# smups/rustronomy-watershed

Hardware: AMD Instinct MI355X
Metric: Mpixels/s segmenting watershed, 8192x8192 u8, device-resident (throughput, 4 transforms of distinct fields in flight; one transform alone: value_one_transform_alone) (higher is better)
Workload: dtype u8 image / u32 stamps+labels (integer min/max/compare); 1 GPU; 8192x8192 u8 uniform[0,254) random field per GPU, segmenting transform, max_water_level 254, seeds = find_local_minima (7320260 on rank 0's first field), engine fused; 4 contexts in flight, each transforming ITS OWN field and seed list (generator seeds 1..4); parallelism=independent fields x1, world_size=1, devices_visible=1, fields_per_gpu=1

## Files before the change

rustronomy-watershed_amd/csrc/ws_common.hpp:

```cpp
#pragma once

#include <hip/hip_runtime.h>
#include <stdint.h>
#include <stdlib.h>

namespace wsk {

#ifdef WS_TUNING
inline const char *tuning_env(const char *name) { return getenv(name); }
#else
inline const char *tuning_env(const char *) { return nullptr; }
#endif

constexpr uint32_t KEY_INF = 0xFF000000u;
constexpr uint32_t RING_MASK = 0x00FFFFFFu;

constexpr int TS = 64;
constexpr int LP = TS + 2;
constexpr int STRIP = 16;
constexpr int NTHREADS = 256;

constexpr int COUNTER_RING = 64;
constexpr int NSTRIPE = 64;
constexpr int STRIPE_STRIDE = 16;
constexpr int FLAG_SLOT = NSTRIPE * STRIPE_STRIDE;

#ifdef __HIPCC__
__device__ __forceinline__ uint32_t wave_inclusive_sum(uint32_t v) {
#define WS_DPP_ADD(ctrl, rows) v += (uint32_t)__builtin_amdgcn_update_dpp(0, (int)v, ctrl, rows, 0xF, false)
  WS_DPP_ADD(0x111, 0xF);
  WS_DPP_ADD(0x112, 0xF);
  WS_DPP_ADD(0x114, 0xF);
  WS_DPP_ADD(0x118, 0xF);
  WS_DPP_ADD(0x142, 0xA);
  WS_DPP_ADD(0x143, 0xC);
#undef WS_DPP_ADD
  return v;
}

__device__ __forceinline__ uint32_t xcd_span_index(uint32_t b, uint32_t n) {
  constexpr uint32_t XCDS = 8;
  const uint32_t per = n / XCDS;
  return b < per * XCDS ? (b % XCDS) * per + b / XCDS : b;
}

__device__ __forceinline__ size_t padded_img_index(int gy, int gx, int W, int SH, size_t stride) {
  const int slice = gy / SH, ry = gy - slice * SH;
  const int iy = max(min(max(ry, 1), SH - 2) - 1, 0), ix = max(min(max(gx, 1), W - 2) - 1, 0);
  return ((size_t)slice * (size_t)max(SH - 2, 0) + iy) * stride + ix;
}
#endif

struct PassFlags {
  uint32_t *edge_changed;
  uint32_t *any_change;
  uint32_t *overflow;
  uint32_t *stats;
};

hipError_t fill_u32(hipStream_t s, uint32_t *p, size_t n, uint32_t v);
hipError_t words_to_host(hipStream_t s, const uint32_t *a, uint32_t na, uint32_t *host_a, const uint32_t *b, uint32_t nb, uint32_t *host_b);
hipError_t zero3(hipStream_t s, uint32_t *a, size_t na, uint32_t *b, size_t nb, uint32_t *c, size_t nc);
hipError_t random_field(hipStream_t s, uint8_t *img, size_t stride, int h, int w, uint64_t seed);
hipError_t scatter_seeds(hipStream_t s, const uint32_t *seeds_rc, const uint32_t *colours, size_t n, int ph, int pw,
                         uint32_t *labels, uint32_t *keys, uint32_t *err_flag);
hipError_t paint_labels(hipStream_t s, const uint32_t *seeds_rc, size_t n, int ph, int pw, uint32_t *labels,
                        uint32_t *err_flag, uint32_t *zero_a, size_t n_zero_a, uint32_t *zero_b, size_t n_zero_b);
hipError_t seed_tables(hipStream_t s, const uint32_t *seeds_rc, size_t n, int ph, int pw, uint32_t *mask, uint32_t *word_base,
                       uint32_t *err_flag, uint32_t *zero_a, size_t n_zero_a, uint32_t *zero_b, size_t n_zero_b,
                       const uint32_t *slice_first = nullptr, size_t slice_px = 0,
                       uint32_t colour_bias = 0);
hipError_t stack_seeds(hipStream_t s, const uint32_t *seeds_rc, size_t n, const uint32_t *slice_first, size_t n_slices,
                       int slice_h, int pw, uint32_t *stacked_rc, uint32_t shift = 0);
hipError_t narrow_seeds(hipStream_t s, const uint64_t *src, size_t n, size_t ph, size_t pw, uint32_t *dst, uint32_t shift = 0);
hipError_t shift_seeds(hipStream_t s, const uint32_t *src, size_t n, uint32_t shift, uint32_t *dst);
hipError_t widen_labels(hipStream_t s, const uint32_t *src, uint64_t *dst, size_t n);
hipError_t snapshot_level(hipStream_t s, const uint32_t *keys, const uint32_t *labels, uint64_t *dst,
                          size_t n, uint32_t level);
hipError_t snapshot_level_u32(hipStream_t s, const uint32_t *keys, const uint32_t *labels, uint32_t *dst, size_t n, uint32_t level);

size_t relax_tiles(int h, int w);
struct RelaxPlane {
  const uint8_t *img = nullptr;
  size_t img_stride = 0;
  uint32_t *keys = nullptr;
  int h = 0, w = 0;
  uint32_t max_level = 0;
  uint32_t *stamps = nullptr;
  PassFlags pf = {};
  uint32_t max_iters = 0xFFFFFFFFu;
  const uint32_t *seed_labels = nullptr;
  bool seed_bits = false;
  int slice_h = 0;
  bool carry_checked_later = false;
  bool padded = false;
  uint32_t *tile_list = nullptr;
  size_t seam_min_px = (size_t)1 << 24;
  int persistent_pass = 0;
};
hipError_t relax_pass(hipStream_t s, const RelaxPlane &plane, uint32_t pass);
struct RelaxPlan;
RelaxPlan relax_plan_for(const RelaxPlane &plane, uint32_t pass);
size_t relax_list_words(int h, int w);

size_t resolve_tiles(int h, int w);
hipError_t resolve_pass(hipStream_t s, const uint32_t *keys, uint32_t *labels, int h, int w,
                        uint32_t pass, uint32_t *stamps, PassFlags pf);
size_t resolve_ref_capacity(int h, int w);
struct ResolveJob {
  const uint32_t *keys = nullptr;
  uint32_t *labels = nullptr;
  int h = 0, w = 0;
  uint32_t *ref_scratch = nullptr;
  uint32_t max_rounds = 0xFFFFFFFFu;
  const uint32_t *seed_mask = nullptr;
  const uint32_t *word_base = nullptr;
  uint32_t *tile_min = nullptr;
  const uint32_t *gate = nullptr;
  uint32_t *carry_flag = nullptr;
  const uint32_t *seed_err = nullptr;
  int halo_flags = 0;
};
hipError_t resolve_two_launch(hipStream_t s, const ResolveJob &job);
hipError_t resolve_chase_again(hipStream_t s, uint32_t *labels, int h, int w, uint32_t *ref_scratch);

hipError_t block_flag_border_tiles(hipStream_t s, uint32_t *stamps, int h, int w, uint32_t pass, int halo_flags);
hipError_t block_export_boundary(hipStream_t s, const uint32_t *labels, int h, int w, int halo_flags, uint32_t rank, uint32_t *rows);
hipError_t block_import_boundary(hipStream_t s, const uint32_t *table, uint32_t world, uint32_t rank, uint32_t *resolved,
                                 uint32_t *labels, int h, int w, int halo_flags);
hipError_t block_iota(hipStream_t s, uint32_t *p, size_t n, uint32_t first);
hipError_t block_rows_differ(hipStream_t s, const uint32_t *a, const uint32_t *b, size_t n, uint32_t *flag);
hipError_t block_pack_cols(hipStream_t s, const uint32_t *plane, size_t h, size_t w, size_t xl, size_t xr, uint32_t *out);
hipError_t block_unpack_cols(hipStream_t s, uint32_t *plane, size_t h, size_t w, const uint32_t *left, const uint32_t *right);

hipError_t flood_step(hipStream_t s, const uint8_t *img, size_t img_stride, const uint32_t *lin,
                      uint32_t *lout, int h, int w, uint32_t level, uint32_t *counter, bool padded = false);

size_t minima_segments(int h, int w);
size_t minima_mask_bytes(int h, int w);
hipError_t minima_count(hipStream_t s, const uint8_t *img, size_t stride, int h, int w, uint32_t *counts, uint8_t *nibbles);
hipError_t minima_write(hipStream_t s, const uint8_t *nibbles, int h, int w, const uint32_t *counts, uint32_t *total, uint32_t *out_rc, size_t cap,
                        uint32_t *mask = nullptr, uint32_t *word_base = nullptr,
                        uint32_t *zero_a = nullptr, size_t n_zero_a = 0, uint32_t *zero_b = nullptr, size_t n_zero_b = 0);
hipError_t widen_pairs(hipStream_t s, const uint32_t *src, uint64_t *dst, size_t n_values);
hipError_t narrow_words(hipStream_t s, const uint64_t *src, uint32_t *dst, size_t n);

inline int tiles_of(int n) { return (n + TS - 1) / TS; }

}
```

rustronomy-watershed_amd/csrc/ws_kernels.hip:

```cpp
#include "ws_common.hpp"

#include <algorithm>
#include <cstdlib>

namespace wsk {


__global__ void k_fill_u32(uint32_t *p, size_t n, uint32_t v) {
  size_t i = (size_t)blockIdx.x * blockDim.x + threadIdx.x;
  const size_t step = (size_t)gridDim.x * blockDim.x;
  for (; i < n; i += step) p[i] = v;
}

hipError_t fill_u32(hipStream_t s, uint32_t *p, size_t n, uint32_t v) {
  if (n == 0) return hipSuccess;
  const int blocks = (int)((n + 1023) / 1024 < 8192 ? (n + 1023) / 1024 : 8192);
  k_fill_u32<<<blocks, 256, 0, s>>>(p, n, v);
  return hipGetLastError();
}

typedef uint32_t u32x4_z __attribute__((ext_vector_type(4)));
__global__ void k_zero3(uint32_t *a, size_t na, uint32_t *b, size_t nb, uint32_t *c, size_t nc) {
  const size_t tid = (size_t)blockIdx.x * blockDim.x + threadIdx.x, step = (size_t)gridDim.x * blockDim.x;
  size_t head = (size_t)((16u - (unsigned)(reinterpret_cast<uintptr_t>(a) & 15u)) & 15u) >> 2;
// ... 411 lines not shown
}

hipError_t widen_pairs(hipStream_t s, const uint32_t *src, uint64_t *dst, size_t n_values) {
  return widen_labels(s, src, dst, n_values);
}

__global__ void k_narrow_words(const uint64_t *__restrict__ src, uint32_t *__restrict__ dst, size_t n) {
  size_t i = (size_t)blockIdx.x * blockDim.x + threadIdx.x;
  const size_t step = (size_t)gridDim.x * blockDim.x;
  for (; i < n; i += step) dst[i] = (uint32_t)src[i];
}

hipError_t narrow_words(hipStream_t s, const uint64_t *src, uint32_t *dst, size_t n) {
  if (n == 0) return hipSuccess;
  const int blocks = (int)((n + 1023) / 1024 < 8192 ? (n + 1023) / 1024 : 8192);
  k_narrow_words<<<blocks, 256, 0, s>>>(src, dst, n);
  return hipGetLastError();
}

__global__ void k_snapshot(const uint32_t *keys, const uint32_t *labels, uint64_t *dst, size_t n,
                           uint32_t level) {
  size_t i = (size_t)blockIdx.x * blockDim.x + threadIdx.x;
  const size_t step = (size_t)gridDim.x * blockDim.x;
  for (; i < n; i += step) {
    const uint32_t k = keys[i];
    dst[i] = (k != KEY_INF && (k >> 24) <= level) ? (uint64_t)labels[i] : 0ull;
  }
}

__global__ void k_snapshot_u32(const uint32_t *__restrict__ keys, const uint32_t *__restrict__ labels, uint32_t *dst, size_t n, uint32_t level) {
  size_t i = (size_t)blockIdx.x * blockDim.x + threadIdx.x;
  const size_t step = (size_t)gridDim.x * blockDim.x;
  for (; i < n; i += step) {
    const uint32_t k = keys[i];
    dst[i] = (k != KEY_INF && (k >> 24) <= level) ? labels[i] : 0u;
  }
}

hipError_t snapshot_level_u32(hipStream_t s, const uint32_t *keys, const uint32_t *labels, uint32_t *dst, size_t n, uint32_t level) {
  if (n == 0) return hipSuccess;
  const int blocks = (int)((n + 1023) / 1024 < 16384 ? (n + 1023) / 1024 : 16384);
  k_snapshot_u32<<<blocks, 256, 0, s>>>(keys, labels, dst, n, level);
  return hipGetLastError();
}

hipError_t snapshot_level(hipStream_t s, const uint32_t *keys, const uint32_t *labels, uint64_t *dst,
                          size_t n, uint32_t level) {
  if (n == 0) return hipSuccess;
  const int blocks = (int)((n + 1023) / 1024 < 8192 ? (n + 1023) / 1024 : 8192);
  k_snapshot<<<blocks, 256, 0, s>>>(keys, labels, dst, n, level);
  return hipGetLastError();
}

__global__ void k_words_to_host(const uint32_t *__restrict__ a, uint32_t na, uint32_t *ha, const uint32_t *__restrict__ b, uint32_t nb,
                                uint32_t *hb) {
  for (uint32_t i = threadIdx.x; i < na; i += blockDim.x) ha[i] = a[i];
  for (uint32_t i = threadIdx.x; i < nb; i += blockDim.x) hb[i] = b[i];
}

hipError_t words_to_host(hipStream_t s, const uint32_t *a, uint32_t na, uint32_t *host_a, const uint32_t *b, uint32_t nb, uint32_t *host_b) {
  k_words_to_host<<<1, 64, 0, s>>>(a, na, host_a, b, nb, host_b);
  return hipGetLastError();
}

typedef uint32_t u32x4_r __attribute__((ext_vector_type(4)));


__device__ __forceinline__ uint32_t pick_drlu(uint32_t d, uint32_t r, uint32_t l, uint32_t u) {
  return d ? d : (r ? r : (l ? l : u));
}

__global__ __launch_bounds__(256) void k_flood_step(const uint8_t *__restrict__ img, size_t img_stride,
                                                    const uint32_t *__restrict__ lin, uint32_t *__restrict__ lout,
                                                    int H, int W, uint32_t level, uint32_t *counter, int pad) {
  const int x = blockIdx.x * 64 + (threadIdx.x & 63);
  const int y = blockIdx.y * 4 + (threadIdx.x >> 6);
  const int xc = min(x, W - 1), yc = min(y, H - 1);
  const int xm = max(xc - 1, 0), xp = min(xc + 1, W - 1), ym = max(yc - 1, 0), yp = min(yc + 1, H - 1);
  const uint32_t c = lin[(size_t)yc * W + xc];
  const uint32_t d = lin[(size_t)yp * W + xc], r = lin[(size_t)yc * W + xp];
  const uint32_t l = lin[(size_t)yc * W + xm], u = lin[(size_t)ym * W + xc];
  const uint32_t v = img[pad ? padded_img_index(yc, xc, W, H, img_stride) : (size_t)yc * img_stride + xc];
  const bool floodable = c == 0u && y >= 1 && y < H - 1 && x >= 1 && x < W - 1 && v <= level;
  const uint32_t pick = floodable ? pick_drlu(d, r, l, u) : 0u;
  if (x < W && y < H) lout[(size_t)y * W + x] = c ? c : pick;
  if (pick && x < W && y < H) *counter = 1u;
}

__global__ __launch_bounds__(256) void k_flood_step4(const uint8_t *__restrict__ img, size_t img_stride,
                                                     const uint32_t *__restrict__ lin, uint32_t *__restrict__ lout,
                                                     int H, int W, uint32_t level, uint32_t *counter) {
  const int y = blockIdx.y;
  const int x0 = (blockIdx.x * 256 + threadIdx.x) * 4;
  if (x0 >= W) return;
  const int ym = max(y - 1, 0), yp = min(y + 1, H - 1);
  const u32x4_r c = *reinterpret_cast<const u32x4_r *>(lin + (size_t)y * W + x0);
  const u32x4_r dn = *reinterpret_cast<const u32x4_r *>(lin + (size_t)yp * W + x0);
  const u32x4_r up = *reinterpret_cast<const u32x4_r *>(lin + (size_t)ym * W + x0);
  const uint32_t lft = lin[(size_t)y * W + max(x0 - 1, 0)], rgt = lin[(size_t)y * W + min(x0 + 4, W - 1)];
  const uint32_t iv = *reinterpret_cast<const uint32_t *>(img + (size_t)y * img_stride + x0);
  const bool row_int = y >= 1 && y < H - 1;
  const uint32_t cc[4] = {c.x, c.y, c.z, c.w}, dd[4] = {dn.x, dn.y, dn.z, dn.w}, uu[4] = {up.x, up.y, up.z, up.w};
  const uint32_t ll[4] = {lft, c.x, c.y, c.z}, rr[4] = {c.y, c.z, c.w, rgt};
  uint32_t out[4], any = 0;
#pragma unroll
  for (int k = 0; k < 4; ++k) {
    const int x = x0 + k;
    const bool floodable = cc[k] == 0u && row_int && x >= 1 && x < W - 1 && ((iv >> (8 * k)) & 0xFFu) <= level;
    const uint32_t pick = floodable ? pick_drlu(dd[k], rr[k], ll[k], uu[k]) : 0u;
    out[k] = cc[k] ? cc[k] : pick;
    any |= pick;
  }
  *reinterpret_cast<u32x4_r *>(lout + (size_t)y * W + x0) = u32x4_r{out[0], out[1], out[2], out[3]};
  if (any) *counter = 1u;
}

// ... 206 lines not shown
```

rustronomy-watershed_amd/csrc/ws_resolve.hip:

```cpp
#include "ws_common.hpp"
#include "ws_resolve_tile.hpp"

#include <algorithm>

namespace wsk {


__device__ __forceinline__ bool tile_must_run(const uint32_t *stamps_prev, int tx, int ty, int tilesX,
                                              int tilesY, uint32_t pass) {
  if (pass == 0) return true;
  const int t = ty * tilesX + tx;
  bool run = false;
  if (ty > 0) run |= stamps_prev[(size_t)(t - tilesX) * 4 + 1] == pass;
  if (ty + 1 < tilesY) run |= stamps_prev[(size_t)(t + tilesX) * 4 + 0] == pass;
  if (tx > 0) run |= stamps_prev[(size_t)(t - 1) * 4 + 3] == pass;
  if (tx + 1 < tilesX) run |= stamps_prev[(size_t)(t + 1) * 4 + 2] == pass;
  return run;
}

size_t resolve_tiles(int h, int w) { return (size_t)tiles_of(w) * tiles_of(h); }


__global__ __launch_bounds__(NTHREADS) void k_resolve(const uint32_t *__restrict__ keys, uint32_t *labels,
                                                      int H, int W, int tilesX, int tilesY, uint32_t pass,
// ... 82 lines not shown
          if (src) { own[i] = src; sB[ly0 + i][lx] = src; todo &= ~(1u << i); changed = 1; changed_mask |= 1u << i; }
        }
      }
    }
    if (!__syncthreads_or(changed)) break;
  }

  if (gx < W) {
#pragma unroll
    for (int i = 0; i < STRIP; ++i) {
      const int gy = gy0 + i;
      if (((changed_mask >> i) & 1u) && gy < H) labels[(size_t)gy * W + gx] = own[i];
    }
  }
  uint32_t e = 0;
  if (strip == 0 && (changed_mask & 1u)) e |= 1u;
  if (strip == (NTHREADS / 64) - 1 && (changed_mask >> (STRIP - 1))) e |= 2u;
  if (lane == 0 && changed_mask) e |= 4u;
  if (lane == 63 && changed_mask) e |= 8u;
  if (changed_mask) e |= 16u;
  if (e) atomicOr(&s_edges, e);
  __syncthreads();
  if (tid == 0) {
    const uint32_t ed = s_edges;
    if (ed) {
      const size_t t = (size_t)tile_y * tilesX + tile_x;
      if (ed & 1u) stamps_cur[t * 4 + 0] = pass + 1;
      if (ed & 2u) stamps_cur[t * 4 + 1] = pass + 1;
      if (ed & 4u) stamps_cur[t * 4 + 2] = pass + 1;
      if (ed & 8u) stamps_cur[t * 4 + 3] = pass + 1;
      const uint32_t stripe = (blockIdx.x % NSTRIPE) * STRIPE_STRIDE;
      if (ed & 15u) pf.edge_changed[(pass % COUNTER_RING) * FLAG_SLOT + stripe] = 1u;
      pf.any_change[stripe] = 1u;
    }
  }
}

hipError_t resolve_pass(hipStream_t s, const uint32_t *keys, uint32_t *labels, int h, int w,
                        uint32_t pass, uint32_t *stamps, PassFlags pf) {
  const int tx = tiles_of(w), ty = tiles_of(h);
  k_resolve<<<tx * ty, NTHREADS, 0, s>>>(keys, labels, h, w, tx, ty, pass, stamps, pf);
  return hipGetLastError();
}


template <bool TABLES, bool MERGE, bool BLOCK>
__global__ __launch_bounds__(NTHREADS, 5) void k_resolve_local(const uint32_t *__restrict__ keys, uint32_t *labels,
                                                            int H, int W, int tilesX, uint32_t *ref_count,
                                                            uint32_t *ref_list, uint32_t max_rounds,
                                                            const uint32_t *__restrict__ seed_mask,
                                                            const uint32_t *__restrict__ word_base, uint32_t *tile_min,
                                                            const uint32_t *__restrict__ gate, int SH, uint32_t *carry_flag,
                                                            const uint32_t *__restrict__ seed_err, int halo_flags) {
  __shared__ __attribute__((aligned(16))) uint32_t sB[RL_ROWS * RL_P];
  if (TABLES && seed_err && (seed_err[0] | seed_err[2]) != 0u) return;
  if (gate && __builtin_amdgcn_ballot_w64(gate[(threadIdx.x & 63) * STRIPE_STRIDE] != 0u) != 0ull) return;
  const uint32_t tile = xcd_span_index(blockIdx.x, gridDim.x);
  const int tile_x = tile % tilesX, tile_y = tile / tilesX;
  const int tid = threadIdx.x;
  const int lane = tid & 63, wave = tid >> 6;
  const int pc = tid & 15, pr = tid >> 4;
  const int x0 = tile_x * TS, y0 = tile_y * TS;
  const int gx0 = x0 + pc * 4, gy0 = y0 + pr * 4;
  const int lx0 = RL_X0 + pc * 4, ly0 = 1 + pr * 4;
  WS_STAMP(0);

  uint32_t K[4][4], Lb[4][4];
  uint32_t seedbits = 0;
  uint32_t tab_mask[4] = {0u, 0u, 0u, 0u}, tab_base[4] = {0u, 0u, 0u, 0u};
  const bool vec = (W & 3) == 0 && ((reinterpret_cast<uintptr_t>(keys) | reinterpret_cast<uintptr_t>(labels)) & 15u) == 0;
  if (vec) {
    const int gxc = min(gx0, W - 4);
    u32x4_r kv[4], lv[4];
#pragma unroll
    for (int r = 0; r < 4; ++r) {
      const size_t g = (size_t)min(gy0 + r, H - 1) * W + gxc;
      kv[r] = *reinterpret_cast<const u32x4_r *>(keys + g);
      if (TABLES) {
        tab_mask[r] = seed_mask[g >> 5];
        tab_base[r] = word_base[g >> 5];
        lv[r] = u32x4_r{0u, 0u, 0u, 0u};
      } else {
        lv[r] = *reinterpret_cast<const u32x4_r *>(labels + g);
      }
    }
#pragma unroll
    for (int r = 0; r < 4; ++r) {
      K[r][0] = kv[r].x; K[r][1] = kv[r].y; K[r][2] = kv[r].z; K[r][3] = kv[r].w;
      Lb[r][0] = lv[r].x; Lb[r][1] = lv[r].y; Lb[r][2] = lv[r].z; Lb[r][3] = lv[r].w;
    }
  } else {
#pragma unroll
    for (int r = 0; r < 4; ++r)
#pragma unroll
      for (int c = 0; c < 4; ++c) {
        const size_t g = (size_t)min(gy0 + r, H - 1) * W + min(gx0 + c, W - 1);
        K[r][c] = keys[g];
        Lb[r][c] = TABLES ? 0u : labels[g];
      }
  }
  {
    const int side = tid >> 6, t = tid & 63;
    const int hy = side == 0 ? y0 - 1 : (side == 1 ? y0 + TS : y0 + t);
    const int hx = side == 2 ? x0 - 1 : (side == 3 ? x0 + TS : x0 + t);
    const size_t hg = (size_t)min(max(hy, 0), H - 1) * W + min(max(hx, 0), W - 1);
    const uint32_t hv = keys[hg];
    const bool hok = hy >= 0 && hy < H && hx >= 0 && hx < W;
    if (!(x0 + TS <= W && y0 + TS <= H)) {
#pragma unroll
      for (int r = 0; r < 4; ++r)
#pragma unroll
        for (int c = 0; c < 4; ++c)
          if (!(gy0 + r < H && gx0 + c < W)) { K[r][c] = KEY_INF; Lb[r][c] = 0u; }
    }
#pragma unroll
    for (int r = 0; r < 4; ++r) {
#pragma unroll
      for (int c = 0; c < 4; ++c)
        if (TABLES && K[r][c] == 0u) seedbits |= 1u << (r * 4 + c);
      *reinterpret_cast<u32x4_r *>(&sB[(ly0 + r) * RL_P + lx0]) = u32x4_r{K[r][0], K[r][1], K[r][2], K[r][3]};
    }
    sB[(hy - (y0 - 1)) * RL_P + (hx - (x0 - 1)) + (RL_X0 - 1)] = hok ? hv : KEY_INF;
  }
  __syncthreads();
  WS_STAMP(1);

  uint32_t P[4][4];
  uint32_t carried = 0u;
  uint32_t live = 0;
  {
    const u32x4_r up4 = *reinterpret_cast<const u32x4_r *>(&sB[(ly0 - 1) * RL_P + lx0]);
    const u32x4_r dn4 = *reinterpret_cast<const u32x4_r *>(&sB[(ly0 + 4) * RL_P + lx0]);
    const uint32_t up[4] = {up4.x, up4.y, up4.z, up4.w}, dn[4] = {dn4.x, dn4.y, dn4.z, dn4.w};
    uint32_t Lc[4], Rc[4];
#pragma unroll
    for (int r = 0; r < 4; ++r) { Lc[r] = sB[(ly0 + r) * RL_P + lx0 - 1]; Rc[r] = sB[(ly0 + r) * RL_P + lx0 + 4]; }
    const uint32_t top_halo = pr == 0, bot_halo = pr == 15, left_halo = pc == 0, right_halo = pc == 15;
    uint32_t row_int[4], col_int[4];
    const int ry0 = SH == H ? gy0 : gy0 % SH;
#pragma unroll
    for (int i = 0; i < 4; ++i) {
      const int ry = ry0 + i >= SH ? ry0 + i - SH : ry0 + i;
      row_int[i] = (uint32_t)(ry >= 1) & (uint32_t)(ry < SH - 1) & (uint32_t)(gy0 + i < H);
      col_int[i] = (uint32_t)(gx0 + i >= 1) & (uint32_t)(gx0 + i < W - 1);
    }
#pragma unroll
    for (int r = 0; r < 4; ++r) {
#pragma unroll
      for (int c = 0; c < 4; ++c) {
        const uint32_t cell = (uint32_t)((ly0 + r) * RL_P + lx0 + c);
        const uint32_t k = K[r][c];
        const uint32_t flood = BLOCK ? (uint32_t)(k - 1u < KEY_INF - 1u) & row_int[r] & col_int[c] : (uint32_t)(k - 1u < KEY_INF - 1u);
        carried = max(carried, flood ? (k - 1u) << 8 : 0u);
        const uint32_t d = r == 3 ? dn[c] : K[r + 1][c];
        const uint32_t rr = c == 3 ? Rc[r] : K[r][c + 1];
        const uint32_t l = c == 0 ? Lc[r] : K[r][c - 1];
        const uint32_t u = r == 0 ? up[c] : K[r - 1][c];
        const uint32_t td = d < k, tr = rr < k, tl = l < k;
        const uint32_t tgt = cell + (uint32_t)(td ? RL_P : (tr ? 1 : (tl ? -1 : -RL_P)));
        const uint32_t kp = td ? d : (tr ? rr : (tl ? l : u));
        uint32_t out_of_tile = 0;
        if (r == 3) out_of_tile |= td & bot_halo;
        if (c == 3) out_of_tile |= (td ^ 1u) & tr & right_halo;
        if (c == 0) out_of_tile |= (td ^ 1u) & (tr ^ 1u) & tl & left_halo;
        if (r == 0) out_of_tile |= (td ^ 1u) & (tr ^ 1u) & (tl ^ 1u) & top_halo;
        const uint32_t fin = (uint32_t)(kp == 0u) | out_of_tile;
        const uint32_t moving = tgt | (fin ? RL_FINAL : 0u) | (out_of_tile ? RL_HALO : 0u);
        P[r][c] = flood ? moving : (cell | RL_FINAL);
        live |= (flood & (fin ^ 1u)) << (r * 4 + c);
      }
    }
  }
  if (carry_flag && carried >= 0xFFFFFE00u) atomicExch(carry_flag, 1u);
  __syncthreads();
#pragma unroll
  for (int r = 0; r < 4; ++r)
    *reinterpret_cast<u32x4_r *>(&sB[(ly0 + r) * RL_P + lx0]) = u32x4_r{P[r][0], P[r][1], P[r][2], P[r][3]};
  __syncthreads();
  WS_STAMP(2);

  for (uint32_t it = 0; live != 0 && it < max_rounds; ++it) {
#pragma unroll
    for (int r = 0; r < 4; ++r)
#pragma unroll
      for (int c = 0; c < 4; ++c) {
        if ((live >> (r * 4 + c)) & 1u) {
          const uint32_t g = sB[P[r][c]];
          P[r][c] = g;
          sB[(ly0 + r) * RL_P + lx0 + c] = g;
          if (g & RL_FINAL) live &= ~(1u << (r * 4 + c));
        }
      }
    WS_STAMP_VALUE(6, it + 1);
  }
  __syncthreads();
  WS_STAMP(3);
  if (TABLES) {
#pragma unroll
    for (int r = 0; r < 4; ++r) {
      const int gyc = min(gy0 + r, H - 1);
      if (vec) {
        const size_t g = (size_t)gyc * W + min(gx0, W - 4);
        asm volatile("" : "+v"(tab_mask[r]), "+v"(tab_base[r]));
        const uint32_t mw = tab_mask[r], wb = tab_base[r], sh = (uint32_t)(g & 31u);
        const uint32_t first = wb + __popc(mw & ((1u << sh) - 1u)) + 1u;
        const uint32_t nib = (seedbits >> (r * 4)) & 15u;
        Lb[r][0] = nib & 1u ? first : 0u;
        Lb[r][1] = nib & 2u ? first + (nib & 1u) : 0u;
        Lb[r][2] = nib & 4u ? first + __popc(nib & 3u) : 0u;
        Lb[r][3] = nib & 8u ? first + __popc(nib & 7u) : 0u;
      } else {
#pragma unroll
        for (int c = 0; c < 4; ++c) {
          const size_t g = (size_t)gyc * W + min(gx0 + c, W - 1);
          const uint32_t col = word_base[g >> 5] + __popc(seed_mask[g >> 5] & ((1u << (g & 31u)) - 1u)) + 1u;
          Lb[r][c] = (seedbits >> (r * 4 + c)) & 1u ? col : 0u;
        }
      }
    }
  }
  if (BLOCK && TABLES) {
#pragma unroll
    for (int r = 0; r < 4; ++r) {
      const int gy = gy0 + r;
      const bool halo_row = (gy == 0 && (halo_flags & 1)) || (gy == H - 1 && (halo_flags & 2));
#pragma unroll
      for (int c = 0; c < 4; ++c)
        if (halo_row && gx0 + c < W && K[r][c] != 0u && K[r][c] != KEY_INF) Lb[r][c] = REF_BIT | (uint32_t)((size_t)gy * W + gx0 + c);
    }
  }
  {
    const int side = tid >> 6, t = tid & 63;
    const int hy = side == 0 ? y0 - 1 : (side == 1 ? y0 + TS : y0 + t);
    const int hx = side == 2 ? x0 - 1 : (side == 3 ? x0 + TS : x0 + t);
    const int hyc = min(max(hy, 0), H - 1), hxc = min(max(hx, 0), W - 1);
    sB[(hy - (y0 - 1)) * RL_P + (hx - (x0 - 1)) + (RL_X0 - 1)] = REF_BIT | (uint32_t)((size_t)hyc * W + hxc);
  }
#pragma unroll
  for (int r = 0; r < 4; ++r)
    *reinterpret_cast<u32x4_r *>(&sB[(ly0 + r) * RL_P + lx0]) = u32x4_r{Lb[r][0], Lb[r][1], Lb[r][2], Lb[r][3]};
  __syncthreads();

  uint32_t refmask = 0;
  uint32_t out[4][4];
#pragma unroll
  for (int r = 0; r < 4; ++r)
#pragma unroll
    for (int c = 0; c < 4; ++c) out[r][c] = sB[P[r][c] & (RL_HALO - 1u)];
  const bool whole = x0 + TS <= W && y0 + TS <= H;
#pragma unroll
  for (int r = 0; r < 4; ++r) {
    const int gy = gy0 + r;
    if (whole) {
#pragma unroll
      for (int c = 0; c < 4; ++c) refmask |= (out[r][c] >> 31) << (r * 4 + c);
    } else {
#pragma unroll
      for (int c = 0; c < 4; ++c)
        refmask |= ((uint32_t)((out[r][c] & REF_BIT) != 0u) & (uint32_t)(gy < H) & (uint32_t)(gx0 + c < W)) << (r * 4 + c);
    }
    if (gy < H) {
      if (vec) {
        if (gx0 < W) *reinterpret_cast<u32x4_r *>(labels + (size_t)gy * W + gx0) = u32x4_r{out[r][0], out[r][1], out[r][2], out[r][3]};
      } else {
#pragma unroll
        for (int c = 0; c < 4; ++c)
          if (gx0 + c < W && (TABLES || (P[r][c] & (RL_HALO - 1u)) != (uint32_t)((ly0 + r) * RL_P + lx0 + c)))
            labels[(size_t)gy * W + gx0 + c] = out[r][c];
      }
    }
  }
  if (MERGE) {
    __shared__ uint32_t sTileLo[NTHREADS / 64], sTileHi[NTHREADS / 64], sTileAny[NTHREADS / 64];
    const bool border_tile = x0 == 0 || y0 == 0 || x0 + TS >= W || y0 + TS >= H;
    uint32_t lo = 0xFFFFFFFFu, hi = 0u;
    bool any_interior = !border_tile;
    if (!border_tile) {
#pragma unroll
      for (int r = 0; r < 4; ++r)
#pragma unroll
        for (int c = 0; c < 4; ++c) { const uint32_t t = out[r][c] - 1u; lo = min(lo, t); hi = max(hi, t); }
    } else {
#pragma unroll
      for (int r = 0; r < 4; ++r)
#pragma unroll
        for (int c = 0; c < 4; ++c) {
          const int gy = gy0 + r, gx = gx0 + c;
          const bool in_plane = gy < H && gx < W;
          const bool inter = gy >= 1 && gy < H - 1 && gx >= 1 && gx < W - 1;
          const bool corner = (gy == 0 || gy == H - 1) && (gx == 0 || gx == W - 1);
          const uint32_t t = out[r][c] - 1u;
          if (in_plane && !corner) lo = min(lo, t);
          if (inter) { hi = max(hi, t); any_interior = true; }
        }
    }
    for (int o = 32; o > 0; o >>= 1) {
      lo = min(lo, (uint32_t)__shfl_xor(lo, o, 64));
      hi = max(hi, (uint32_t)__shfl_xor(hi, o, 64));
    }
    const bool wave_any = __ballot(any_interior) != 0ull;
    if (lane == 0) { sTileLo[wave] = lo; sTileHi[wave] = hi; sTileAny[wave] = wave_any ? 1u : 0u; }
    __syncthreads();
    if (tid == 0) {
      uint32_t l = sTileLo[0], h2 = sTileHi[0], a = sTileAny[0];
#pragma unroll
      for (int k = 1; k < NTHREADS / 64; ++k) { l = min(l, sTileLo[k]); h2 = max(h2, sTileHi[k]); a |= sTileAny[k]; }
      const bool one_lake = h2 != 0xFFFFFFFFu && a != 0u;
      tile_min[tile] = !one_lake ? 0u : (l < REF_BIT - 1u ? l + 1u : RL_TILE_UNDECIDED);
    }
  }
  WS_STAMP(4);
  const uint32_t cnt = __popc(refmask);
  const uint32_t incl = wave_inclusive_sum(cnt);
  const size_t region = (size_t)blockIdx.x * (NTHREADS / 64) + wave;
  const bool all_refs = (uint32_t)__builtin_amdgcn_readlane((int)incl, 63) >= REF_DENSE;
  if (lane == 63) ref_count[region] = all_refs ? REF_ALL : incl;
  if (refmask && !all_refs) {
    uint2 *dst = reinterpret_cast<uint2 *>(ref_list) + region * REF_REGION + (incl - cnt);
#pragma unroll
    for (int i = 0; i < 16; ++i)
      if ((refmask >> i) & 1u) *dst++ = make_uint2((uint32_t)((size_t)(gy0 + (i >> 2)) * W + gx0 + (i & 3)), out[i >> 2][i & 3] & ~REF_BIT);
  }
  WS_STAMP(5);
}

__global__ __launch_bounds__(256) void k_resolve_chase(uint32_t *labels, const uint32_t *__restrict__ ref_count,
                                const uint32_t *__restrict__ ref_list, size_t nregions, size_t n,
                                const uint32_t *__restrict__ gate, const uint32_t *__restrict__ seed_err,
                                size_t follow_from, size_t follow_to, int H, int W, int tilesX, uint32_t ntiles, int halve) {
  const int lane = threadIdx.x & 63;
  if (seed_err && (seed_err[0] | seed_err[2]) != 0u) return;
  if (gate && __builtin_amdgcn_ballot_w64(gate[lane * STRIPE_STRIDE] != 0u) != 0ull) return;
  const size_t wave0 = ((size_t)blockIdx.x * blockDim.x + threadIdx.x) >> 6, nwaves = ((size_t)gridDim.x * blockDim.x) >> 6;
  const size_t ngroups = (nregions + CH_R - 1) / CH_R;
  const size_t span = follow_to - follow_from;
  for (size_t grp = wave0; grp < ngroups; grp += nwaves) {
    const size_t r0 = (ngroups - 1 - grp) * CH_R;
    uint32_t cnt = 0;
    if (lane < CH_R && r0 + lane < nregions) cnt = ref_count[r0 + lane];
    const unsigned long long all_refs = __builtin_amdgcn_ballot_w64(cnt == REF_ALL);
    cnt = cnt == REF_ALL ? 0u : min(cnt, (uint32_t)REF_REGION);
    const uint32_t incl = wave_inclusive_sum(cnt);
    const uint32_t tot = (uint32_t)__builtin_amdgcn_readlane((int)incl, 63);
    uint32_t ends[CH_R - 1];
#pragma unroll
    for (int i = 0; i < CH_R - 1; ++i) ends[i] = (uint32_t)__builtin_amdgcn_readlane((int)incl, i);
    for (uint32_t jb = 0; jb < tot; jb += 64 * CH_U) {
      uint2 e[CH_U];
      uint32_t v[CH_U];
      bool ok[CH_U];
#pragma unroll
      for (int u = 0; u < CH_U; ++u) {
        const uint32_t j = jb + u * 64 + lane;
        ok[u] = j < tot;
        uint32_t reg = 0, base = 0;
#pragma unroll
        for (int i = 0; i < CH_R - 1; ++i)
          if (j >= ends[i]) { reg = i + 1; base = ends[i]; }
        e[u] = reinterpret_cast<const uint2 *>(ref_list)[(r0 + (ok[u] ? reg : 0u)) * REF_REGION + (ok[u] ? j - base : 0u)];
      }
      bool follow[CH_U];
      uint32_t first[CH_U];
#pragma unroll
      for (int u = 0; u < CH_U; ++u) {
        v[u] = e[u].y | REF_BIT;
        follow[u] = ok[u] && n != 0 && (size_t)e[u].y - follow_from < span;
        first[u] = __hip_atomic_load(labels + (follow[u] ? e[u].y : (uint32_t)follow_from), __ATOMIC_RELAXED, __HIP_MEMORY_SCOPE_AGENT);
      }
#pragma unroll
      for (int u = 0; u < CH_U; ++u) {
        if (follow[u]) v[u] = follow_chain<false>(labels, first[u], follow_from, span, n);
      }
#pragma unroll
      for (int u = 0; u < CH_U; ++u)
        if (ok[u]) labels[e[u].x] = v[u];
    }
    for (unsigned long long m = all_refs; m != 0ull; m &= m - 1ull) {
      const size_t region = r0 + (size_t)__builtin_ctzll(m);
      const uint32_t tile = xcd_span_index((uint32_t)(region / (NTHREADS / 64)), ntiles);
      const int gx0 = (int)(tile % (uint32_t)tilesX) * TS + (lane & 15) * 4;
      const int gy0 = (int)(tile / (uint32_t)tilesX) * TS + ((int)(region % (NTHREADS / 64)) * 4 + (lane >> 4)) * 4;
      const bool vec = (W & 3) == 0 && (reinterpret_cast<uintptr_t>(labels) & 15u) == 0;
// ... 45 lines not shown
          if (gy0 + r < H && gx0 < W) *reinterpret_cast<u32x4_r *>(labels + (size_t)(gy0 + r) * W + gx0) = u32x4_r{L[r][0], L[r][1], L[r][2], L[r][3]};
      } else {
#pragma unroll
        for (int r = 0; r < 4; ++r)
#pragma unroll
          for (int c = 0; c < 4; ++c)
            if (gy0 + r < H && gx0 + c < W) labels[(size_t)(gy0 + r) * W + gx0 + c] = L[r][c];
      }
    }
  }
}

size_t resolve_ref_capacity(int h, int w) {
  const size_t nregions = (size_t)tiles_of(w) * tiles_of(h) * (NTHREADS / 64);
  return nregions * (1 + 2 * REF_REGION);
}

static unsigned chase_grid(size_t nregions) { return (unsigned)std::min<size_t>(((nregions + CH_R - 1) / CH_R + 3) / 4, 4096); }

template <bool TABLES, bool MERGE, bool BLOCK>
static hipError_t launch_resolve_local(hipStream_t s, const ResolveJob &j, int halo_rows) {
  const int tx = tiles_of(j.w), ty = tiles_of(j.h);
  uint32_t *ref_count = j.ref_scratch, *ref_list = j.ref_scratch + (size_t)tx * ty * (NTHREADS / 64);
  k_resolve_local<TABLES, MERGE, BLOCK><<<tx * ty, NTHREADS, 0, s>>>(j.keys, j.labels, j.h, j.w, tx, ref_count, ref_list, j.max_rounds,
                                                                    TABLES ? j.seed_mask : nullptr, TABLES ? j.word_base : nullptr,
                                                                    MERGE ? j.tile_min : nullptr, j.gate,  j.h, j.carry_flag,
                                                                    TABLES ? j.seed_err : nullptr, BLOCK && TABLES ? halo_rows : 0);
  return hipGetLastError();
}

hipError_t resolve_two_launch(hipStream_t s, const ResolveJob &job) {
  const int tx = tiles_of(job.w), ty = tiles_of(job.h);
  const size_t n = (size_t)job.h * job.w;
  if (n == 0) return hipSuccess;
  const size_t nregions = (size_t)tx * ty * (NTHREADS / 64);
  const bool tables = job.seed_mask != nullptr;
  const bool ring = !tables && (job.halo_flags & 4) != 0;
  const int halo_rows = job.halo_flags & 3;
  const bool block = ring || (tables && halo_rows != 0);
  const bool merge = !block && job.tile_min != nullptr;
  hipError_t e = hipErrorInvalidValue;
  switch ((tables ? 4 : 0) | (merge ? 2 : 0) | (block ? 1 : 0)) {
    case 0: e = launch_resolve_local<false, false, false>(s, job, halo_rows); break;
    case 1: e = launch_resolve_local<false, false, true>(s, job, halo_rows); break;
    case 2: e = launch_resolve_local<false, true, false>(s, job, halo_rows); break;
    case 4: e = launch_resolve_local<true, false, false>(s, job, halo_rows); break;
    case 5: e = launch_resolve_local<true, false, true>(s, job, halo_rows); break;
    case 6: e = launch_resolve_local<true, true, false>(s, job, halo_rows); break;
  }
  if (e != hipSuccess) return e;
  const size_t from = (halo_rows & 1) ? (size_t)job.w : 0, to = (halo_rows & 2) ? n - (size_t)job.w : n;
  k_resolve_chase<<<chase_grid(nregions), 256, 0, s>>>(job.labels, job.ref_scratch, job.ref_scratch + nregions, nregions, n, job.gate,
                                                       tables ? job.seed_err : nullptr, from, to, job.h, job.w, tx, (uint32_t)(tx * ty),
                                                       halo_rows == 0 && !ring ? 1 : 0);
  return hipGetLastError();
}

hipError_t resolve_chase_again(hipStream_t s, uint32_t *labels, int h, int w, uint32_t *ref_scratch) {
  const size_t n = (size_t)h * w;
  if (n == 0) return hipSuccess;
  const size_t nregions = (size_t)tiles_of(w) * tiles_of(h) * (NTHREADS / 64);
  k_resolve_chase<<<chase_grid(nregions), 256, 0, s>>>(labels, ref_scratch, ref_scratch + nregions, nregions, n, nullptr, nullptr, 0, n, h, w, tiles_of(w), (uint32_t)(tiles_of(w) * tiles_of(h)), 0);
  return hipGetLastError();
}

}
```

rustronomy-watershed_amd/csrc/ws_segment.hip:

```cpp
#include "ws_ctx.hpp"
#include "ws_relax_plan.hpp"

#include <atomic>
#include <mutex>
#include <system_error>
#include <thread>

namespace wsapi {

int run_fused_form(ws_ctx *c, const uint8_t *d_img, size_t stride, int ph, int pw, uint32_t max_level,
                   const uint32_t *d_seeds, size_t n_seeds, uint32_t *d_labels, bool tables, bool *mispredicted,
                   int slice_h, const uint32_t *slice_first, bool padded, MinimaSeeds *minima) {
  const size_t n = (size_t)ph * pw;
  const size_t ntiles = (size_t)tiles_of(pw) * tiles_of(ph);
  const size_t nwords = (n + 31) / 32;
  int rc;
  if ((rc = ensure(c, c->keys, (n ? n : 1) * sizeof(uint32_t)))) return rc;
  if ((rc = ensure(c, c->stamps, std::max(ntiles, relax_tiles(ph, pw)) * 4 * 2 * sizeof(uint32_t)))) return rc;
  if (tables && (rc = ensure(c, c->seed_tab, (nwords ? nwords : 1) * 2 * sizeof(uint32_t)))) return rc;
  if ((rc = ensure(c, c->tile_list, relax_list_words(ph, pw) * sizeof(uint32_t)))) return rc;
  if (minima && (rc = ensure(c, c->min_counts, std::max<size_t>(minima_segments(ph, pw), 1) * sizeof(uint32_t)))) return rc;
  if (minima && (rc = ensure(c, c->min_nibbles, std::max<size_t>(minima_mask_bytes(ph, pw), 1)))) return rc;
  uint32_t *tile_list = (uint32_t *)c->tile_list.p;
  uint32_t *keys = (uint32_t *)c->keys.p;
// ... 19 lines not shown
  key.stride = stride; key.n_seeds = n_seeds; key.ph = ph; key.pw = pw; key.slice_h = slice_h; key.padded = padded; key.max_level = max_level;
  key.generation = c->buffer_generation;
  key.from_minima = minima != nullptr;
  key.persist_mode = persist_mode;
  if (minima) { key.seeds = minima->d_list; key.n_seeds = minima->cap; }
  auto resolve_job = [&](const uint32_t *gate) {
    ResolveJob job;
    job.keys = keys; job.labels = d_labels; job.h = ph; job.w = pw;
    job.ref_scratch = (uint32_t *)c->refs.p; job.max_rounds = c->debug_max_iters;
    job.seed_mask = seed_mask; job.word_base = word_base; job.seed_err = flags + FLAG_SEED_ERR;
    job.tile_min = c->tile_min_out;
    job.gate = gate;
    job.carry_flag = flags + FLAG_OVERFLOW;
    return job;
  };
  auto make_tables = [&]() -> hipError_t {
    if (!minima)
      return seed_tables(c->stream, d_seeds, n_seeds, ph, pw, seed_mask, word_base, flags + FLAG_SEED_ERR, stamps,
                         relax_tiles(ph, pw) * 4 * 2, flags, FLAG_MISC, slice_first, (size_t)slice_h * pw);
    uint32_t *counts = (uint32_t *)c->min_counts.p;
    uint8_t *nibbles = (uint8_t *)c->min_nibbles.p;
    hipError_t e = minima_count(c->stream, d_img, stride, ph, pw, counts, nibbles);
    if (e == hipSuccess)
      e = minima_write(c->stream, nibbles, ph, pw, counts, flags + FLAG_TOTAL, minima->d_list, minima->cap, seed_mask, word_base, stamps, relax_tiles(ph, pw) * 4 * 2, flags, FLAG_MISC);
    return e;
  };
  const bool graph_ok = use_graph && c->stream != nullptr && !c->graph_unusable && tables && n != 0 && n < 0x80000000ull && !c->profiling && c->misc_clean &&
                        c->debug_max_iters == 0xFFFFFFFFu;
  const bool resume = c->async_phase == ws_ctx::ASYNC_RESUME;
  if (resume) c->async_phase = ws_ctx::ASYNC_NONE;
  if (resume) graph_mode = 1;
  else if (graph_ok && c->graph_exec && key == c->graph_key) graph_mode = 1;
  else if (graph_ok && key == c->seen_key) graph_mode = 2;
  if (!resume) c->seen_key = graph_ok ? key : ws_ctx::GraphKey();
  if (graph_mode != 0) {
    if ((rc = ensure(c, c->refs, resolve_ref_capacity(ph, pw) * sizeof(uint32_t)))) return rc;
    if (c->buffer_generation != key.generation && !resume) graph_mode = 0;
  }
  if (graph_mode == 2) {
    if (c->graph_exec) { (void)hipGraphExecDestroy(c->graph_exec); c->graph_exec = nullptr; }
    if (hipStreamBeginCapture(c->stream, hipStreamCaptureModeThreadLocal) != hipSuccess) {
      (void)hipGetLastError();
      c->graph_unusable = true;
      graph_mode = 0;
    }
  }
  if (graph_mode == 2) {
    RelaxPlane captured = plane;
    captured.pf = make_pf(c); captured.seed_labels = seed_mask; captured.seed_bits = true; captured.carry_checked_later = true;
    hipGraph_t graph = nullptr;
    hipError_t e = make_tables();
    for (uint32_t pass = 0; pass < GRAPH_PASSES && e == hipSuccess; ++pass) e = relax_pass(c->stream, captured, pass);
    const uint32_t last = GRAPH_PASSES - 1;
    if (e == hipSuccess)
      e = resolve_two_launch(c->stream, resolve_job(edge_slot(flags, last)));
    if (e == hipSuccess && c->pinned_dev)
      e = words_to_host(c->stream, edge_slot(flags, last), FLAG_SLOT, c->pinned_dev + FLAG_EDGE + (last % COUNTER_RING) * FLAG_SLOT,
                        flags + FLAG_OVERFLOW, FLAG_NERR + 1, c->pinned_dev + FLAG_OVERFLOW);
    if (e == hipSuccess && !c->pinned_dev)
      e = hipMemcpyAsync(&c->pinned[FLAG_EDGE + (last % COUNTER_RING) * FLAG_SLOT], edge_slot(flags, last), FLAG_SLOT * sizeof(uint32_t),
                         hipMemcpyDeviceToHost, c->stream);
    if (e == hipSuccess && !c->pinned_dev)
      e = hipMemcpyAsync(&c->pinned[FLAG_OVERFLOW], flags + FLAG_OVERFLOW, (FLAG_NERR + 1) * sizeof(uint32_t), hipMemcpyDeviceToHost, c->stream);
    const hipError_t e2 = hipStreamEndCapture(c->stream, &graph);
    if (e == hipSuccess && e2 == hipSuccess) e = hipGraphInstantiate(&c->graph_exec, graph, nullptr, nullptr, 0);
    if (graph) (void)hipGraphDestroy(graph);
    if (e != hipSuccess || e2 != hipSuccess) {
      (void)hipGetLastError();
      c->graph_exec = nullptr;
      c->graph_unusable = true;
      graph_mode = 0;
    } else {
      c->graph_key = key;
    }
  }
  if (graph_mode != 0) {
    c->have_keys = false;
    *mispredicted = false;
    c->misc_clean = false;
    c->stats.graph_launches = 1;
    if (!resume) HIP_TRY(c, hipGraphLaunch(c->graph_exec, c->stream));
    if (c->async_phase == ws_ctx::ASYNC_BEGIN && graph_mode == 1) {
      HIP_TRY(c, hipEventRecord(c->async_ev, c->stream));
      c->async_phase = ws_ctx::ASYNC_LAUNCHED;
      return WS_INTERNAL_PENDING;
    }
    if (resume) HIP_TRY(c, hipEventSynchronize(c->async_ev));
    else HIP_TRY(c, hipStreamSynchronize(c->stream));
  } else {
    Span sp(c, KC_OTHER);
    if (!c->misc_clean) HIP_TRY(c, hipMemsetAsync(flags + FLAG_OVERFLOW, 0, FLAG_NERR * sizeof(uint32_t), c->stream));
    c->misc_clean = false;
    if (tables)
      HIP_TRY(c, make_tables());
    else
      HIP_TRY(c, paint_labels(c->stream, d_seeds, n_seeds, ph, pw, d_labels, flags + FLAG_SEED_ERR, stamps,
                              relax_tiles(ph, pw) * 4 * 2, flags, FLAG_MISC));
  }
  if (n == 0) return WS_OK;

  const PassFlags pf = make_pf(c);
  const bool two_launch = n < 0x80000000ull;
  static const bool no_speculation = tuning_env("WS_NO_SPECULATION") != nullptr;
  if (two_launch && (rc = ensure(c, c->refs, resolve_ref_capacity(ph, pw) * sizeof(uint32_t)))) return rc;
  auto resolve = [&](const uint32_t *gate) -> int {
    Span sp(c, KC_RESOLVE);
    HIP_TRY(c, resolve_two_launch(c->stream, resolve_job(gate)));
    return WS_OK;
  };
  uint32_t speculated_after = 0xFFFFFFFFu, converged_at = 0xFFFFFFFFu;
  std::function<int(uint32_t)> speculate = nullptr;
// ... 545 lines not shown
```

Measured before the change: 172,100 Mpixels/s.

## Fold flag readback into resolve chase kernel and precompute halo seed colours

Drops the separate single-block words_to_host kernel. Block 0 of k_resolve_chase now copies the edge flags and overflow words to pinned host memory, which removes one launch from the captured graph. The resolve-local kernel also computes seed colours for halo cells from the seed tables, so halo cells that are unlabelled seeds get their colour directly instead of a reference to chase. This costs extra shared memory and a moved barrier. The readback now runs at the start of the chase kernel, which may be earlier than the flags are final if that kernel does not write them.

```diff
diff --git a/rustronomy-watershed_amd/csrc/ws_common.hpp b/rustronomy-watershed_amd/csrc/ws_common.hpp
--- a/rustronomy-watershed_amd/csrc/ws_common.hpp
+++ b/rustronomy-watershed_amd/csrc/ws_common.hpp
@@ -59,7 +59,6 @@
 };
 
 hipError_t fill_u32(hipStream_t s, uint32_t *p, size_t n, uint32_t v);
-hipError_t words_to_host(hipStream_t s, const uint32_t *a, uint32_t na, uint32_t *host_a, const uint32_t *b, uint32_t nb, uint32_t *host_b);
 hipError_t zero3(hipStream_t s, uint32_t *a, size_t na, uint32_t *b, size_t nb, uint32_t *c, size_t nc);
 hipError_t random_field(hipStream_t s, uint8_t *img, size_t stride, int h, int w, uint64_t seed);
 hipError_t scatter_seeds(hipStream_t s, const uint32_t *seeds_rc, const uint32_t *colours, size_t n, int ph, int pw,
@@ -107,6 +106,11 @@
 hipError_t resolve_pass(hipStream_t s, const uint32_t *keys, uint32_t *labels, int h, int w,
                         uint32_t pass, uint32_t *stamps, PassFlags pf);
 size_t resolve_ref_capacity(int h, int w);
+struct ReadBack {
+  const uint32_t *src = nullptr;
+  uint32_t count = 0;
+  uint32_t *host = nullptr;
+};
 struct ResolveJob {
   const uint32_t *keys = nullptr;
   uint32_t *labels = nullptr;
@@ -119,6 +123,7 @@
   const uint32_t *gate = nullptr;
   uint32_t *carry_flag = nullptr;
   const uint32_t *seed_err = nullptr;
+  ReadBack read_back[2];
   int halo_flags = 0;
 };
 hipError_t resolve_two_launch(hipStream_t s, const ResolveJob &job);
diff --git a/rustronomy-watershed_amd/csrc/ws_kernels.hip b/rustronomy-watershed_amd/csrc/ws_kernels.hip
--- a/rustronomy-watershed_amd/csrc/ws_kernels.hip
+++ b/rustronomy-watershed_amd/csrc/ws_kernels.hip
@@ -487,16 +487,6 @@
   return hipGetLastError();
 }
 
-__global__ void k_words_to_host(const uint32_t *__restrict__ a, uint32_t na, uint32_t *ha, const uint32_t *__restrict__ b, uint32_t nb,
-                                uint32_t *hb) {
-  for (uint32_t i = threadIdx.x; i < na; i += blockDim.x) ha[i] = a[i];
-  for (uint32_t i = threadIdx.x; i < nb; i += blockDim.x) hb[i] = b[i];
-}
-
-hipError_t words_to_host(hipStream_t s, const uint32_t *a, uint32_t na, uint32_t *host_a, const uint32_t *b, uint32_t nb, uint32_t *host_b) {
-  k_words_to_host<<<1, 64, 0, s>>>(a, na, host_a, b, nb, host_b);
-  return hipGetLastError();
-}
 
 typedef uint32_t u32x4_r __attribute__((ext_vector_type(4)));
 
diff --git a/rustronomy-watershed_amd/csrc/ws_resolve.hip b/rustronomy-watershed_amd/csrc/ws_resolve.hip
--- a/rustronomy-watershed_amd/csrc/ws_resolve.hip
+++ b/rustronomy-watershed_amd/csrc/ws_resolve.hip
@@ -158,7 +158,7 @@
                                                             const uint32_t *__restrict__ word_base, uint32_t *tile_min,
                                                             const uint32_t *__restrict__ gate, int SH, uint32_t *carry_flag,
                                                             const uint32_t *__restrict__ seed_err, int halo_flags) {
-  __shared__ __attribute__((aligned(16))) uint32_t sB[RL_ROWS * RL_P];
+  __shared__ __attribute__((aligned(16))) uint32_t sB[RL_ROWS * RL_P + (TABLES && !BLOCK ? NTHREADS : 0)];
   if (TABLES && seed_err && (seed_err[0] | seed_err[2]) != 0u) return;
   if (gate && __builtin_amdgcn_ballot_w64(gate[(threadIdx.x & 63) * STRIPE_STRIDE] != 0u) != 0ull) return;
   const uint32_t tile = xcd_span_index(blockIdx.x, gridDim.x);
@@ -172,6 +172,8 @@
   WS_STAMP(0);
 
   uint32_t K[4][4], Lb[4][4];
+  constexpr bool HALO_SEEDS = TABLES && !BLOCK;
+  uint32_t *const sHaloColour = sB + RL_ROWS * RL_P;
   uint32_t seedbits = 0;
   uint32_t tab_mask[4] = {0u, 0u, 0u, 0u}, tab_base[4] = {0u, 0u, 0u, 0u};
   const bool vec = (W & 3) == 0 && ((reinterpret_cast<uintptr_t>(keys) | reinterpret_cast<uintptr_t>(labels)) & 15u) == 0;
@@ -212,6 +214,8 @@
     const size_t hg = (size_t)min(max(hy, 0), H - 1) * W + min(max(hx, 0), W - 1);
     const uint32_t hv = keys[hg];
     const bool hok = hy >= 0 && hy < H && hx >= 0 && hx < W;
+    uint32_t hmask = 0u, hbase = 0u;
+    if (HALO_SEEDS && vec && side < 2) { hmask = seed_mask[hg >> 5]; hbase = word_base[hg >> 5]; }
     if (!(x0 + TS <= W && y0 + TS <= H)) {
 #pragma unroll
       for (int r = 0; r < 4; ++r)
@@ -227,6 +231,7 @@
       *reinterpret_cast<u32x4_r *>(&sB[(ly0 + r) * RL_P + lx0]) = u32x4_r{K[r][0], K[r][1], K[r][2], K[r][3]};
     }
     sB[(hy - (y0 - 1)) * RL_P + (hx - (x0 - 1)) + (RL_X0 - 1)] = hok ? hv : KEY_INF;
+    if (HALO_SEEDS && vec && side < 2) sHaloColour[tid] = hbase + __popc(hmask & ((1u << (hg & 31u)) - 1u)) + 1u;
   }
   __syncthreads();
   WS_STAMP(1);
@@ -299,9 +304,10 @@
       }
     WS_STAMP_VALUE(6, it + 1);
   }
-  __syncthreads();
+  if (!HALO_SEEDS) __syncthreads();
   WS_STAMP(3);
   if (TABLES) {
+    uint32_t side_first[4] = {0u, 0u, 0u, 0u};
 #pragma unroll
     for (int r = 0; r < 4; ++r) {
       const int gyc = min(gy0 + r, H - 1);
@@ -315,6 +321,7 @@
         Lb[r][1] = nib & 2u ? first + (nib & 1u) : 0u;
         Lb[r][2] = nib & 4u ? first + __popc(nib & 3u) : 0u;
         Lb[r][3] = nib & 8u ? first + __popc(nib & 7u) : 0u;
+        if (HALO_SEEDS) side_first[r] = first;
       } else {
 #pragma unroll
         for (int c = 0; c < 4; ++c) {
@@ -324,7 +331,14 @@
         }
       }
     }
-  }
+    if (HALO_SEEDS && vec && (pc == 0 || pc == 15)) {
+      uint32_t cand[4];
+#pragma unroll
+      for (int r = 0; r < 4; ++r) cand[r] = pc == 0 ? side_first[r] - 1u : side_first[r] + __popc((seedbits >> (r * 4)) & 15u);
+      *reinterpret_cast<u32x4_r *>(&sHaloColour[(pc == 0 ? 128 : 192) + pr * 4]) = u32x4_r{cand[0], cand[1], cand[2], cand[3]};
+    }
+  }
+  if (HALO_SEEDS) __syncthreads();
   if (BLOCK && TABLES) {
 #pragma unroll
     for (int r = 0; r < 4; ++r) {
@@ -340,7 +354,12 @@
     const int hy = side == 0 ? y0 - 1 : (side == 1 ? y0 + TS : y0 + t);
     const int hx = side == 2 ? x0 - 1 : (side == 3 ? x0 + TS : x0 + t);
     const int hyc = min(max(hy, 0), H - 1), hxc = min(max(hx, 0), W - 1);
-    sB[(hy - (y0 - 1)) * RL_P + (hx - (x0 - 1)) + (RL_X0 - 1)] = REF_BIT | (uint32_t)((size_t)hyc * W + hxc);
+    if (HALO_SEEDS && vec) {
+      const int cell = (hy - (y0 - 1)) * RL_P + (hx - (x0 - 1)) + (RL_X0 - 1);
+      sB[cell] = sB[cell] == 0u ? sHaloColour[tid] : REF_BIT | (uint32_t)((size_t)hyc * W + hxc);
+    } else {
+      sB[(hy - (y0 - 1)) * RL_P + (hx - (x0 - 1)) + (RL_X0 - 1)] = REF_BIT | (uint32_t)((size_t)hyc * W + hxc);
+    }
   }
 #pragma unroll
   for (int r = 0; r < 4; ++r)
@@ -433,7 +452,12 @@
 __global__ __launch_bounds__(256) void k_resolve_chase(uint32_t *labels, const uint32_t *__restrict__ ref_count,
                                 const uint32_t *__restrict__ ref_list, size_t nregions, size_t n,
                                 const uint32_t *__restrict__ gate, const uint32_t *__restrict__ seed_err,
-                                size_t follow_from, size_t follow_to, int H, int W, int tilesX, uint32_t ntiles, int halve) {
+                                size_t follow_from, size_t follow_to, int H, int W, int tilesX, uint32_t ntiles, int halve,
+                                ReadBack rb0, ReadBack rb1) {
+  if (blockIdx.x == 0) {
+    for (uint32_t i = threadIdx.x; i < rb0.count; i += blockDim.x) rb0.host[i] = rb0.src[i];
+    for (uint32_t i = threadIdx.x; i < rb1.count; i += blockDim.x) rb1.host[i] = rb1.src[i];
+  }
   const int lane = threadIdx.x & 63;
   if (seed_err && (seed_err[0] | seed_err[2]) != 0u) return;
   if (gate && __builtin_amdgcn_ballot_w64(gate[lane * STRIPE_STRIDE] != 0u) != 0ull) return;
@@ -585,7 +609,7 @@
   const size_t from = (halo_rows & 1) ? (size_t)job.w : 0, to = (halo_rows & 2) ? n - (size_t)job.w : n;
   k_resolve_chase<<<chase_grid(nregions), 256, 0, s>>>(job.labels, job.ref_scratch, job.ref_scratch + nregions, nregions, n, job.gate,
                                                        tables ? job.seed_err : nullptr, from, to, job.h, job.w, tx, (uint32_t)(tx * ty),
-                                                       halo_rows == 0 && !ring ? 1 : 0);
+                                                       halo_rows == 0 && !ring ? 1 : 0, job.read_back[0], job.read_back[1]);
   return hipGetLastError();
 }
 
@@ -593,7 +617,8 @@
   const size_t n = (size_t)h * w;
   if (n == 0) return hipSuccess;
   const size_t nregions = (size_t)tiles_of(w) * tiles_of(h) * (NTHREADS / 64);
-  k_resolve_chase<<<chase_grid(nregions), 256, 0, s>>>(labels, ref_scratch, ref_scratch + nregions, nregions, n, nullptr, nullptr, 0, n, h, w, tiles_of(w), (uint32_t)(tiles_of(w) * tiles_of(h)), 0);
+  k_resolve_chase<<<chase_grid(nregions), 256, 0, s>>>(labels, ref_scratch, ref_scratch + nregions, nregions, n, nullptr, nullptr, 0, n, h, w, tiles_of(w), (uint32_t)(tiles_of(w) * tiles_of(h)), 0,
+                                                       ReadBack(), ReadBack());
   return hipGetLastError();
 }
 
diff --git a/rustronomy-watershed_amd/csrc/ws_segment.hip b/rustronomy-watershed_amd/csrc/ws_segment.hip
--- a/rustronomy-watershed_amd/csrc/ws_segment.hip
+++ b/rustronomy-watershed_amd/csrc/ws_segment.hip
@@ -95,11 +95,13 @@
     hipError_t e = make_tables();
     for (uint32_t pass = 0; pass < GRAPH_PASSES && e == hipSuccess; ++pass) e = relax_pass(c->stream, captured, pass);
     const uint32_t last = GRAPH_PASSES - 1;
+    ResolveJob job = resolve_job(edge_slot(flags, last));
+    if (c->pinned_dev) {
+      job.read_back[0] = {edge_slot(flags, last), (uint32_t)FLAG_SLOT, c->pinned_dev + FLAG_EDGE + (last % COUNTER_RING) * FLAG_SLOT};
+      job.read_back[1] = {flags + FLAG_OVERFLOW, (uint32_t)(FLAG_NERR + 1), c->pinned_dev + FLAG_OVERFLOW};
+    }
     if (e == hipSuccess)
-      e = resolve_two_launch(c->stream, resolve_job(edge_slot(flags, last)));
-    if (e == hipSuccess && c->pinned_dev)
-      e = words_to_host(c->stream, edge_slot(flags, last), FLAG_SLOT, c->pinned_dev + FLAG_EDGE + (last % COUNTER_RING) * FLAG_SLOT,
-                        flags + FLAG_OVERFLOW, FLAG_NERR + 1, c->pinned_dev + FLAG_OVERFLOW);
+      e = resolve_two_launch(c->stream, job);
     if (e == hipSuccess && !c->pinned_dev)
       e = hipMemcpyAsync(&c->pinned[FLAG_EDGE + (last % COUNTER_RING) * FLAG_SLOT], edge_slot(flags, last), FLAG_SLOT * sizeof(uint32_t),
                          hipMemcpyDeviceToHost, c->stream);
```

Result: faster. 179,800 Mpixels/s (median of 6 runs) (+4.5%).
